# crowsonkb/style-transfer-pytorch

Measured on AMD Instinct MI355X. Metric: optimizer iterations/sec, higher is better.
Workload: dtype f32 (3x3 convs: fp16x3 split-plane MFMA, fp32 accumulate); 1 GPU; 512x512 single-scale hot loop (closure + Adam + clamp + EMA), 1 style image 512x512, VGG-19 synthetic weights, max pooling; parallelism=single GPU

## Files before the change

style-transfer-pytorch_amd/csrc/st_closure.hip:

```cpp
#include <cmath>
#include <cstdlib>
#include <mutex>

#include "st_plan.h"

namespace st {

void conv_arithmetic(const st_net* net, int conv, bool dgrad, ConvProblem& c) {
    const bool wide = dgrad ? net->wide_bwd[conv] : net->wide_fwd[conv];
    if (wide) {
        c.wgt_split = dgrad ? net->wsx_bwd[conv] : net->wsx_fwd[conv];
        c.planes = 3;
        c.elem = 0;
    } else {
        c.wgt_split = dgrad ? net->ws_bwd[conv] : net->ws_fwd[conv];
        c.planes = net->conv_planes;
        c.elem = net->conv_elem;
    }
}

int plan_alloc(st_plan* p, float** out, size_t floats) {
    void* ptr = nullptr;
    const size_t bytes = ((floats * sizeof(float) + 255) / 256) * 256;
    hipError_t e = hipMalloc(&ptr, bytes);
// ... 226 lines not shown
                StyleHead& h0 = p->head[0];
                static Option fwd_too("ST_CONV1_GRAM_IN_FORWARD", 0);
                p->gram1_fused = (fork_heads || fwd_too.get() != 0) && last_layer >= 1 && bounds && p->reference_taps && h0.allocated &&
                                 conv_first_gram_applies(p->H, p->W, image, n.y, h0.gram.max_splits);
                if (hbm_profiled(p, HBM_CONV1_FWD, (3 + 64) * hw4, s, [&] {
                        if (p->gram1_fused)
                            return launch_conv_first_fwd_gram(image, net->w_first, net->bias[0], n.y, p->H, p->W, s, n.y_amax,
                                                              h0.gram.partial, h0.gram.partial_sum, h0.gram.max_splits,
                                                              &p->gram1_splits, net->w_first_l1max, net->b_first_max);
                        return launch_conv_first_fwd(image, net->w_first, net->bias[0], n.y, p->H, p->W, s, nullptr, 0, 0,
                                                     bounds ? n.y_amax : nullptr);
                    }))
                    return 1;
            } else {
                ConvProblem c{};
                forward_conv(p, i, c);
                if (pool_follows(p, i, last_layer)) c.pool_out = p->pool[kProgram[i + 1].index].y;
                pooled_by_conv = fuse_pool(c, n, fork_heads, nullptr);
                if (conv_launch_profiled(p, c, s)) return 1;
            }
            prev = &n;
            if (fork_heads) {
                for (int k = 0; k < p->n_style; ++k)
                    if (p->style_op[k] == i) ST_HIP(hipEventRecord(p->tap_ready[k], s));
            }
        } else {
            Node& n = p->pool[op.index];
            if (!pooled_by_conv && launch_pool_fwd(prev->y, n.y, prev->c, prev->h, prev->w, net->pooling, s)) return 1;
            pooled_by_conv = false;
            prev = &n;
        }
    }
    return 0;
}

int ensure_moment_alloc(st_plan* p, StyleHead& h) {
    if (h.allocated) return 0;
    const size_t nn = (size_t)h.n * h.n;
    if (plan_alloc(p, &h.srm, nn) || plan_alloc(p, &h.ssym, nn) || plan_alloc(p, &h.mean, h.n) || plan_alloc(p, &h.bvec, h.n))
        return 1;
    long long splits = (16ll << 20) / (long long)nn;
    if (splits > 1024) splits = 1024;
    if (splits < 8) splits = 8;
    h.gram.max_splits = (int)splits;
    if (plan_alloc(p, &h.gram.partial, (size_t)splits * nn) ||
        plan_alloc(p, &h.gram.partial_sum, (size_t)splits * h.n))
        return 1;
    const long long wg = ((h.npix_local + 255) / 256) * (h.n / 64);
    if (wg < 512) {
        size_t need = (size_t)(h.n / 32) * h.n * (size_t)h.npix_local;
        if (need > kConvScratchFloats) need = kConvScratchFloats;
        if (plan_alloc(p, &h.conv_scratch, need)) return 1;
    }
    h.allocated = true;
    return 0;
}

int ensure_style_alloc(st_plan* p, StyleHead& h) {
    if (ensure_moment_alloc(p, h)) return 1;
    const size_t nn = (size_t)h.n * h.n;
    if (p->style_kind == 1) return h.gram_t ? 0 : plan_alloc(p, &h.gram_t, nn);
    if (h.w2_allocated) return 0;
    float** mats[] = {&h.cov_t, &h.root_t, &h.cov, &h.tmat, &h.mmat, &h.root, &h.gm, &h.dt, &h.dcov};
    for (float** m : mats)
        if (!*m && plan_alloc(p, m, nn)) return 1;
    if ((!h.mean_t && plan_alloc(p, &h.mean_t, h.n)) || (!h.gdiag && plan_alloc(p, &h.gdiag, 64))) return 1;
    float* nsbase = nullptr;
    if (plan_alloc(p, &nsbase, ns_workspace_floats(h.n))) return 1;
    ns_workspace_carve(h.ns, nsbase, h.n);
    if (ns_workspace_reset(h.ns, nullptr)) return 1;
// ... 20 lines not shown

HeadSite head_site(st_plan* p, int j) {
    HeadSite at;
    const int op = p->style_op[j];
    Node& tap = node_at(p, op);
    at.h = &p->head[op];
    at.tap = &tap;
    at.weight = p->style_weight[j];
    at.loss = p->losses + 1 + j;
    at.grad = tap.g;
    at.grad_amax = tap.g_amax;
    at.slot = j;
    return at;
}

int moments_of_tap(st_plan* p, const HeadSite& at, float* mean_out, float* srm_out, hipStream_t s, float* cov_out) {
    StyleHead& h = *at.h;
    const Node& tap = *at.tap;
    const int idx = at.slot;
    const bool fused = idx == 0 && p->gram1_fused;
    const int splits = fused ? p->gram1_splits : gram_choose_splits(h.n, h.npix_local, h.gram.max_splits);
    static Option gram_f32("ST_GRAM_F32", 0);
    auto gram = [&] {
        if (!fused && !(ablate_side() & 1) &&
            launch_gram_partial(tap.y, h.n, h.npix_local, splits, h.gram, s,
                                (p->net->conv_elem == 1 && !gram_f32.get()) ? tap.y_amax : nullptr))
            return 1;
        return launch_gram_finalize(h.gram, h.n, h.npix, splits, mean_out, srm_out, s, cov_out, kCovEps);
    };
    if (idx == 0 && !fused) return hbm_profiled(p, HBM_GRAM1, 4.0 * h.n * (double)h.npix_local, s, gram);
    return gram();
}

int moment_sums_of_tap(st_plan* p, int j, float* sums, hipStream_t s) {
    StyleHead& h = p->head[p->style_op[j]];
    const Node& tap = node_at(p, p->style_op[j]);
    const int splits = gram_choose_splits(h.n, h.npix_local, h.gram.max_splits);
    if (launch_gram_partial(tap.y, h.n, h.npix_local, splits, h.gram, s, p->net->conv_elem == 1 ? tap.y_amax : nullptr))
        return 1;
    return launch_gram_finalize(h.gram, h.n, 1, splits, sums + (size_t)h.n * h.n, sums, s);
}

GemmBatch one_gemm(int n, const float* a, const float* b, float* d, int ta, int tb) {
    GemmBatch g{};
    g.n = n; g.count = 1;
    g.p[0].a1 = a; g.p[0].b1 = b; g.p[0].d = d; g.p[0].ta1 = ta; g.p[0].tb1 = tb;
    g.p[0].epilogue = EPI_SCALE; g.p[0].c = 1.f;
    return g;
}

// ... 32 lines not shown
    if (launch_gemm_batch(mm, s)) return 1;
    const W2LossJob job{h.mean, h.mean_t, h.cov, h.cov_t, h.root, n, w, at.loss, h.gdiag};
    if (idx >= 0 && ns_chain_combined() && (ns_chain_mask() & (idx == 4 ? 4 : idx == 3 ? 2 : 1))) {
        const float* mm1[1] = {h.mmat};
        float* r1[1] = {h.root};
        float* g1[1] = {h.gm};
        NSWorkspace* w1[1] = {&h.ns};
        if (ns_chain_delayed() && idx != 4) ST_HIP(hipStreamWaitEvent(s, p->aux_fwd, 0));
        if (ns_sqrt_chain(mm1, r1, g1, &n, w1, &m_partials, &job, 1, s)) return 1;
        if (tl) ST_HIP(hipEventRecord(tlh[1], s));
    } else {
        int root_partials = 0;
        if (ns_sqrt_forward(h.mmat, h.root, n, h.ns, s, m_partials, &root_partials)) return 1;
        if (tl) ST_HIP(hipEventRecord(tlh[1], s));
        if (ns_sqrt_backward(h.root, nullptr, h.gdiag, h.gm, n, h.ns, s, &job, root_partials)) return 1;
    }
    if (tl) ST_HIP(hipEventRecord(tlh[2], s));
    if (launch_gemm_batch(one_gemm(n, h.gm, h.root_t, h.dt, 0, 1), s)) return 1;
    if (launch_gemm_batch(one_gemm(n, h.root_t, h.dt, h.dcov, 1, 0), s)) return 1;
    const bool f16 = p->net->conv_elem == 1;
    return launch_style_grad_finish(h.dcov, h.mean, h.mean_t, n, w, h.npix, h.ssym, h.bvec, s, f16 ? h.s_amax : nullptr);
}

int style_heads_shallow_lockstep(st_plan* p, hipStream_t s, const int* idx, int lanes) {
    const bool with_cov = gram_fused_cov();
    StyleHead* h[3];
    HeadSite at[3];
    int n[3];
    static Option defer_opt("ST_GRAM_DEFER_PIXELS", 0);
    const bool defer = defer_opt.get() > 0 && (long long)p->H * p->W >= defer_opt.get();
    for (int l = 0; l < lanes; ++l) {
        at[l] = head_site(p, idx[l]);
        h[l] = at[l].h;
        n[l] = h[l]->n;
        ST_HIP(hipStreamWaitEvent(s, defer ? p->aux_fwd : p->tap_ready[idx[l]], 0));
        if (moments_of_tap(p, at[l], h[l]->mean, h[l]->srm, s, with_cov ? h[l]->cov : nullptr)) return 1;
        if (!with_cov && launch_cov_from_moments(h[l]->mean, h[l]->srm, h[l]->cov, n[l], kCovEps, s)) return 1;
    }
    auto batch3 = [&](auto make) {
        GemmBatch g{};
        g.n = 64; g.count = lanes;
        for (int l = 0; l < lanes; ++l) g.n = std::max(g.n, n[l]);
        for (int l = 0; l < lanes; ++l) {
            g.p[l] = make(l);
            g.p[l].n = n[l];
        }
        return launch_gemm_batch(g, s);
    };
    if (batch3([&](int l) { return one_gemm(n[l], h[l]->root_t, h[l]->cov, h[l]->tmat, 0, 0).p[0]; })) return 1;
    if (batch3([&](int l) { return one_gemm(n[l], h[l]->tmat, h[l]->root_t, h[l]->mmat, 0, 0).p[0]; })) return 1;
    const float* mm[3] = {};
    float* roots[3] = {};
    NSWorkspace* ws[3] = {};
    for (int l = 0; l < lanes; ++l) { mm[l] = h[l]->mmat; roots[l] = h[l]->root; ws[l] = &h[l]->ns; }
    W2LossJob jobs[3];
    for (int l = 0; l < lanes; ++l)
        jobs[l] = W2LossJob{h[l]->mean, h[l]->mean_t, h[l]->cov, h[l]->cov_t, h[l]->root, n[l], at[l].weight, at[l].loss, h[l]->gdiag};
    const float* croots[3] = {};
// ... 41 lines not shown
        c.planes = 2; c.elem = 1; c.amax_word = tap.y_amax; c.wgt_amax = h.s_amax;
    }
    c.scratch = h.conv_scratch;
    if (idx == 4 && head5_masks_its_gradient()) c.out_mask = tap.y;
    if (ablate_side() & 2) return 0;
    const long long npix = (long long)tap.h * tap.w;
    if (head_dgrad_small_applies(n, npix))
        return hbm_profiled(p, HBM_HEAD_1X1, 2.0 * n * (double)npix * sizeof(float), s, [&] {
            return launch_head_dgrad_small(h.ssym, tap.y, h.bvec, c.out_mask, at.grad, n, npix, c.out_amax, s);
        });
    return hbm_profiled(p, HBM_HEAD_1X1, 2.0 * n * (double)tap.h * tap.w * sizeof(float), s, [&] { return launch_conv(c, s); });
}

bool op_is_tap(const st_plan* p, int op) {
    for (int i = 0; i < p->n_content; ++i)
        if (p->content_op[i] == op) return true;
    for (int k = 0; k < p->n_style; ++k)
        if (p->style_op[k] == op) return true;
    return false;
}

int join_head_for_conv(st_plan* p, int conv_index, hipStream_t s) {
    for (int k = 0; k < p->n_style; ++k) {
        if (!head_taps_conv(p, k, conv_index)) continue;
        ST_HIP(hipStreamWaitEvent(s, p->head_done[k], 0));
    }
    return 0;
}

void dgrad_conv(const st_plan* p, int i, ConvProblem& c) {
    const st_net* net = p->net;
    const OpDesc& op = kProgram[i];
    const OpDesc& pop = kProgram[i - 1];
    const Node& n = p->conv[op.index];
    const Node& in = node_at(p, i - 1);
    const bool top = i == kNumOps - 1;
    c.in = n.g; c.mask = (top && !head5_masks_its_gradient()) ? n.y : nullptr;
    c.out_mask = (pop.kind == 0) ? in.y : nullptr;
    c.wgt = net->w_bwd[op.index]; c.bias = nullptr; c.out = in.g;
    c.cin = op.cout; c.cout = op.cin; c.height = n.h; c.width = n.w; c.taps = 9; c.relu = 0;
    c.accumulate = (pop.kind == 0 && op_is_tap(p, i - 1)) ? 1 : 0;
    c.scratch = p->conv_scratch;
    conv_arithmetic(net, op.index, true, c);
    c.amax_word = n.g_amax; c.out_amax = net->conv_elem == 1 ? in.g_amax : nullptr;
}

int run_backward(st_plan* p, float* grad_image, hipStream_t s) {
// ... 99 lines not shown
    return 0;
}

int loss_and_grad(st_plan* p, const float* image, float* grad_out, float* losses_out, hipStream_t s) {
    if (require_targets(p) || ensure_grad_alloc(p)) return 1;
    if (ensure_streams(p, s)) return 1;
    if (p->timeline) ST_HIP(hipEventRecord(p->tl_start, s));
    auto tv = [&](hipStream_t ts) {
        return hbm_profiled(p, HBM_TV, 2.0 * 3 * 4.0 * p->H * p->W, ts, [&] {
            return launch_tv(image, p->H, p->W, p->tv_weight, grad_out, p->red_partials, p->losses + 6, ts, p->tickets + 0);
        });
    };
    static Option tv_slot_opt("ST_TV_SLOT", 0);
    const bool tv_tail = tv_slot_opt.get() == 1 && !p->aux_stream;
    if (!tv_tail) {
        const int tvk = shallow_heads_lockstep(p) ? 2 : 0;
        if (!p->aux_stream && ensure_head_stream(p, tvk)) return 1;
        hipStream_t tvs = p->aux_stream ? p->aux_stream : p->head_stream[tvk];
        ST_HIP(hipEventRecord(p->aux_in, s));
        ST_HIP(hipStreamWaitEvent(tvs, p->aux_in, 0));
        if (tv(tvs)) return 1;
        ST_HIP(hipEventRecord(p->tv_done, tvs));
    }
    if (run_forward(p, image, 29, s, true)) return 1;
    if (p->timeline) ST_HIP(hipEventRecord(p->tl_fwd, s));
    const int cop = p->content_op[0];
    Node& ct = node_at(p, cop);
    ST_HIP(hipEventRecord(p->aux_fwd, s));
    auto content = [&](hipStream_t cstream) {
        ST_HIP(hipStreamWaitEvent(cstream, p->aux_fwd, 0));
        if (hbm_profiled(p, HBM_CONTENT, 3.0 * 4.0 * ct.count(), cstream, [&] {
                return launch_content_mse(ct.y, p->content_target[cop], (long long)ct.count(), p->content_weight[0], ct.g,
                                          p->red_partials + 4 * kStreamBlocks, p->losses + 0, cstream, p->tickets + 64);
            }))
            return 1;
        ST_HIP(hipEventRecord(p->content_done, cstream));
        return 0;
    };
    if (p->aux_stream && content(p->aux_stream)) return 1;
    const bool lockstep = shallow_heads_lockstep(p);
    for (int k = 4; k >= (lockstep ? 3 : 0); --k) {
        const bool on_caller = k == 4 && p->head4_on_caller;
        if (!on_caller && ensure_head_stream(p, k)) return 1;
        hipStream_t hs = on_caller ? s : p->head_stream[k];
        if (!on_caller) ST_HIP(hipStreamWaitEvent(hs, p->tap_ready[k], 0));
        if (style_head(p, head_site(p, k), hs)) return 1;
        ST_HIP(hipEventRecord(p->head_done[k], hs));
        if (p->timeline) ST_HIP(hipEventRecord(p->tl_head[k], hs));
        if (k == 3 && !p->aux_stream && content(p->head_stream[3])) return 1;
    }
    if (lockstep) {
        const int three[3] = {2, 1, 0};
        if (ensure_head_stream(p, 2) || style_heads_shallow_lockstep(p, p->head_stream[2], three, 3)) return 1;
    }
    if (tv_tail) {
        hipStream_t tvs = p->head_stream[lockstep ? 2 : 0];
        if (tv(tvs)) return 1;
        ST_HIP(hipEventRecord(p->tv_done, tvs));
    }
    if (run_backward(p, grad_out, s)) return 1;
    if (!p->defer_sum && launch_sum_losses(p->losses, s, losses_out)) return 1;
    if (p->timeline) {
        ST_HIP(hipEventRecord(p->tl_bwd, s));
        if (++p->tl_count % 10 == 0) {
            ST_HIP(hipEventSynchronize(p->tl_bwd));
            float f = 0, b = 0, h[5] = {};
            hipEventElapsedTime(&f, p->tl_start, p->tl_fwd);
            hipEventElapsedTime(&b, p->tl_start, p->tl_bwd);
            for (int i = 0; i < 5; ++i) hipEventElapsedTime(&h[i], p->tl_start, p->tl_head[i]);
            float c4[3] = {};
            for (int i = 0; i < 3; ++i) hipEventElapsedTime(&c4[i], p->tl_start, p->tl_h4[i]);
            fprintf(stderr, "[timeline] relu5_1 head: moments known %.3f | NS forward done %.3f | NS backward done %.3f | gradient written %.3f ms\n",
                    c4[0], c4[1], c4[2], h[4]);
            float c3[3] = {};
            for (int i = 0; i < 3; ++i) hipEventElapsedTime(&c3[i], p->tl_start, p->tl_h3[i]);
// ... 56 lines not shown
```

style-transfer-pytorch_amd/csrc/st_common.h:

```cpp
#pragma once

#include <hip/hip_runtime.h>

#include <algorithm>
#include <atomic>
#include <cstdarg>
#include <cstdio>
#include <string>

namespace st {

typedef float f32x16 __attribute__((ext_vector_type(16)));
typedef float f32x4 __attribute__((ext_vector_type(4)));
typedef float f32x2 __attribute__((ext_vector_type(2)));

constexpr int kWave = 64;

void set_error(const char* fmt, ...);
const char* get_error();

#define ST_HIP(expr)                                                                           \
    do {                                                                                       \
        hipError_t _e = (expr);                                                                \
        if (_e != hipSuccess) {                                                                \
// ... 40 lines not shown
        const unsigned long long c = cached.load(std::memory_order_acquire);
        if ((unsigned)(c >> 32) == g) return (int)(unsigned)(c & 0xffffffffull);
        const int v = option_lookup(name, dflt);
        cached.store(((unsigned long long)g << 32) | (unsigned)v, std::memory_order_release);
        return v;
    }
};

__device__ __forceinline__ float wave_sum(float v) {
#pragma unroll
    for (int off = 32; off > 0; off >>= 1) v += __shfl_xor(v, off, 64);
    return v;
}

__device__ __forceinline__ float block_sum_256(float v, float* scratch) {
    v = wave_sum(v);
    const int lane = threadIdx.x & 63, wave = threadIdx.x >> 6;
    if (lane == 0) scratch[wave] = v;
    __syncthreads();
    float r = 0.f;
    if (threadIdx.x == 0) r = (scratch[0] + scratch[1]) + (scratch[2] + scratch[3]);
    __syncthreads();
    return r;
}

struct W2LossJob {
    const float *mean, *mean_t, *cov, *cov_t, *root;
    int n;
    float weight;
    float* loss_out;
    float* gdiag_out;
};
__device__ __forceinline__ float w2_gdiag(const W2LossJob& j) { return -2.f * (j.weight / (float)j.n); }
__device__ __forceinline__ void w2_loss_block(const W2LossJob& j, float* scratch) {
#pragma clang fp contract(off)
    float sm = 0.f, sc = 0.f;
    for (int i = threadIdx.x; i < j.n; i += 256) {
        const float d = j.mean[i] - j.mean_t[i];
        sm += d * d;
        const size_t ii = (size_t)i * j.n + i;
        sc += (j.cov_t[ii] + j.cov[ii]) - 2.f * j.root[ii];
    }
    sm = block_sum_256(sm, scratch);
    sc = block_sum_256(sc, scratch);
    if (threadIdx.x == 0) {
        const float fn = (float)j.n;
// ... 139 lines not shown

int launch_pool_fwd(const float* in, float* out, int channels, int height, int width, int mode, hipStream_t s);
bool conv_pc_fuses_pool(const ConvProblem& p);
int fold_halo_amax(const ConvProblem& p, hipStream_t stream);
struct PcOverlap {
    int rows_b;
    int rows_bottom;
    int shape_i, tw_i;
    int shape_b, tw_b;
    double cost_split, cost_whole;
    bool pays;
    bool pool;
};
bool conv_pc_overlap_choice(const ConvProblem& p, PcOverlap* out);
int launch_pool_bwd_codes(const unsigned char* code, const float* grad_out, float* grad_in, int channels, int height,
                          int width, hipStream_t s);
int launch_pool_bwd(const float* in, const float* grad_out, float* grad_in, int channels, int height,
                    int width, int mode, hipStream_t s);

struct GramWorkspace {
    float* partial;
    float* partial_sum;
    int max_splits;
};
int gram_choose_splits(int channels, long long npix, int max_splits);
int launch_gram_partial(const float* feat, int channels, long long npix, int splits, GramWorkspace ws,
                        hipStream_t s, const unsigned int* bound = nullptr);
int launch_gram_finalize(GramWorkspace ws, int channels, long long npix, int splits, float* mean, float* srm,
                         hipStream_t s, float* cov = nullptr, float cov_eps = 0.f);

enum GemmEpilogue {
    EPI_SCALE = 0,
    EPI_IDENT_MINUS = 1,
    EPI_DIFF = 2,
    EPI_DEV_SQRT_SCALE = 3
};
struct GemmProblem {
    const float* a1; const float* b1;
    const float* a2; const float* b2; const float* b2sub;
    float* d;
    int ta1, tb1, ta2;
    int epilogue;
    float c, ci;
    const float* dev_scalar;
    int n;
    float* sumsq_partials;
};
bool gemm_sumsq_fusable(int n);
struct GemmBatch {
    GemmProblem p[6];
    int count;
    int n;
// ... 220 lines not shown
```

style-transfer-pytorch_amd/csrc/st_gram.hip:

```cpp
#include "st_common.h"

namespace st {
namespace {

constexpr int GT = 64;
constexpr int GK = 64;
constexpr int GP = 68;
constexpr int HK = 32;
constexpr int HP = 40;

typedef _Float16 f16x8 __attribute__((ext_vector_type(8)));

__device__ __forceinline__ void tile_pair(int block, int tiles, int& ti, int& tj) {
    int t = block, row = 0, len = tiles;
    while (t >= len) {
        t -= len;
        --len;
        ++row;
    }
    ti = row;
    tj = row + t;
}

__device__ __forceinline__ void store_tile_pair(float* __restrict__ out, int C, int ti, int tj, int wi, int wj,
// ... 94 lines not shown
            const f32x4 a = *reinterpret_cast<const f32x4*>(la + kb * 8);
            const f32x4 b = *reinterpret_cast<const f32x4*>(lb + kb * 8);
#pragma unroll
            for (int e = 0; e < 4; ++e) acc = __builtin_amdgcn_mfma_f32_32x32x2f32(a[e], b[e], acc, 0, 0, 0);
        }
        if (more) store_tile(buf ^ 1);
        __syncthreads();
    }

    store_tile_pair(partial + (size_t)split * C * C, C, ti, tj, wi, wj, l31, half, acc);
    if (diag) {
#pragma unroll
        for (int r = 0; r < 4; ++r) {
            float v = rowsum[r];
            v += __shfl_xor(v, 1, 64);
            v += __shfl_xor(v, 2, 64);
            v += __shfl_xor(v, 4, 64);
            v += __shfl_xor(v, 8, 64);
            if ((tid & 15) == 0) partial_sum[(size_t)split * C + ti * GT + srow + 16 * r] = v;
        }
    }
}

__global__ __launch_bounds__(256) void gram_partial_f16_kernel(const float* __restrict__ feat, int C, long long N,
                                                               int splits, long long per_split,
                                                               const unsigned int* __restrict__ bound,
                                                               float* __restrict__ partial,
                                                               float* __restrict__ partial_sum, int xcd_remap) {
    __shared__ __attribute__((aligned(16))) _Float16 lds[2][2][2][GT * HP];
    const int tid = threadIdx.x, lane = tid & 63;
    const int wave = __builtin_amdgcn_readfirstlane(tid >> 6);
    const int l31 = lane & 31, half = lane >> 5;
    const int wi = wave >> 1, wj = wave & 1;
    const int tiles = C / GT;
    int ti, tj;
    const unsigned int lb = logical_block(xcd_remap);
    tile_pair((int)(lb % gridDim.x), tiles, ti, tj);
    const int split = (int)(lb / gridDim.x);
    const long long k_begin = split * per_split;
    const long long k_end = (k_begin + per_split < N) ? k_begin + per_split : N;
    const bool diag = (ti == tj);
    const bool vec_ok = (N % 4 == 0);
    const int ex = scale_exp(amax_read(bound));
    const float scale = pow2f(ex), unscale = pow2f(-ex);

    const int srow = tid >> 2, scol = (tid & 3) * 8;
    float va[8], vb[8];
    float rowsum = 0.f;

    auto load_row = [&](const float* p, long long k, float (&v)[8]) {
#pragma unroll
        for (int q = 0; q < 2; ++q) {
            if (vec_ok && k + 4 * q + 3 < k_end) {
                const f32x4 t = *reinterpret_cast<const f32x4*>(p + 4 * q);
#pragma unroll
                for (int e = 0; e < 4; ++e) v[4 * q + e] = t[e];
            } else {
#pragma unroll
                for (int e = 0; e < 4; ++e) v[4 * q + e] = (k + 4 * q + e < k_end) ? p[4 * q + e] : 0.f;
            }
        }
    };
    auto load_tile = [&](long long k0) {
        const long long k = k0 + scol;
        load_row(feat + (size_t)(ti * GT + srow) * N + k, k, va);
        if (!diag) load_row(feat + (size_t)(tj * GT + srow) * N + k, k, vb);
    };
    auto split_store = [&](const float (&v)[8], _Float16* p0, _Float16* p1) {
        f16x8 h0, h1;
#pragma unroll
        for (int e = 0; e < 8; ++e) {
            const float x = v[e] * scale;
            const _Float16 a = (_Float16)x;
            h0[e] = a;
            h1[e] = (_Float16)(x - (float)a);
        }
        *reinterpret_cast<f16x8*>(p0) = h0;
        *reinterpret_cast<f16x8*>(p1) = h1;
    };
    auto store_tile = [&](int buf) {
        const int off = srow * HP + scol;
        split_store(va, &lds[buf][0][0][off], &lds[buf][0][1][off]);
        if (!diag) split_store(vb, &lds[buf][1][0][off], &lds[buf][1][1][off]);
        rowsum += ((va[0] + va[1]) + (va[2] + va[3])) + ((va[4] + va[5]) + (va[6] + va[7]));
    };

    f32x16 acc;
#pragma unroll
    for (int r = 0; r < 16; ++r) acc[r] = 0.f;

    const long long span = k_end - k_begin;
    const int nstages = span > 0 ? (int)((span + HK - 1) / HK) : 0;
    if (nstages > 0) {
        load_tile(k_begin);
        store_tile(0);
    }
    __syncthreads();
    const int ob = diag ? 0 : 1;
    for (int st = 0; st < nstages; ++st) {
        const int buf = st & 1;
        const bool more = st + 1 < nstages;
        if (more) load_tile(k_begin + (long long)(st + 1) * HK);
        const int aoff = (wi * 32 + l31) * HP + 8 * half, boff = (wj * 32 + l31) * HP + 8 * half;
#pragma unroll
        for (int kb = 0; kb < HK / 16; ++kb) {
            const f16x8 a0 = *reinterpret_cast<const f16x8*>(&lds[buf][0][0][aoff + kb * 16]);
            const f16x8 a1 = *reinterpret_cast<const f16x8*>(&lds[buf][0][1][aoff + kb * 16]);
// ... 2 lines not shown
            acc = __builtin_amdgcn_mfma_f32_32x32x16_f16(a0, b0, acc, 0, 0, 0);
            acc = __builtin_amdgcn_mfma_f32_32x32x16_f16(a0, b1, acc, 0, 0, 0);
            acc = __builtin_amdgcn_mfma_f32_32x32x16_f16(a1, b0, acc, 0, 0, 0);
        }
        if (more) store_tile(buf ^ 1);
        __syncthreads();
    }
#pragma unroll
    for (int r = 0; r < 16; ++r) acc[r] = acc[r] * unscale * unscale;
    float* out = partial + (size_t)split * C * C;
    if (diag) {
        float* t = reinterpret_cast<float*>(&lds[0][0][0][0]);
#pragma unroll
        for (int r = 0; r < 16; ++r)
            t[(wi * 32 + (r & 3) + 8 * (r >> 2) + 4 * half) * 65 + wj * 32 + l31] = acc[r];
        __syncthreads();
        for (int idx = tid; idx < GT * GT; idx += 256) {
            const int row = idx >> 6, col = idx & 63;
            out[(size_t)(ti * GT + row) * C + ti * GT + col] = row <= col ? t[row * 65 + col] : t[col * 65 + row];
        }
    } else {
        store_tile_pair(out, C, ti, tj, wi, wj, l31, half, acc);
    }
    if (diag) {
        float v = rowsum;
        v += __shfl_xor(v, 1, 64);
        v += __shfl_xor(v, 2, 64);
        if ((tid & 3) == 0) partial_sum[(size_t)split * C + ti * GT + srow] = v;
    }
}

__global__ __launch_bounds__(256, 2) void gram_partial_f16_wide_kernel(const float* __restrict__ feat, int C, long long N,
                                                                       int splits, long long per_split,
                                                                       const unsigned int* __restrict__ bound,
                                                                       float* __restrict__ partial,
                                                                       float* __restrict__ partial_sum, int xcd_remap) {
    constexpr int TS = 128;
    __shared__ __attribute__((aligned(16))) _Float16 lds[2][2][TS * HP];
    const int tid = threadIdx.x, lane = tid & 63;
    const int wave = __builtin_amdgcn_readfirstlane(tid >> 6);
    const int l31 = lane & 31, half = lane >> 5;
    const int wi = wave >> 1, wj = wave & 1;
    int ti, tj;
    const unsigned int lb = logical_block(xcd_remap);
    tile_pair((int)(lb % gridDim.x), C / TS, ti, tj);
    const int split = (int)(lb / gridDim.x);
    const long long k_begin = split * per_split;
    const long long k_end = (k_begin + per_split < N) ? k_begin + per_split : N;
    const bool diag = (ti == tj);
    const bool vec_ok = (N % 4 == 0);
    const int ex = scale_exp(amax_read(bound));
// ... 196 lines not shown
    if (want > by_len) want = by_len;
    if (want > max_splits) want = max_splits;
    if (want < 1) want = 1;
    return (int)want;
}

int launch_gram_partial(const float* feat, int channels, long long npix, int splits, GramWorkspace ws,
                        hipStream_t s, const unsigned int* bound) {
    ST_REQUIRE(channels % GT == 0, "gram: channel count must be a multiple of 64");
    ST_REQUIRE(splits >= 1 && splits <= ws.max_splits, "gram: bad split count %d", splits);
    long long per_split = (npix + splits - 1) / splits;
    per_split = (per_split + 3) & ~3ll;
    static Option remap_opt("ST_XCD_REMAP", 1);
    const int remap = remap_opt.get();
    if (bound && gram_wide_tiles(channels, npix)) {
        const int wide = (channels / 128) * (channels / 128 + 1) / 2;
        hipLaunchKernelGGL(gram_partial_f16_wide_kernel, dim3(wide, splits), dim3(256), 0, s, feat, channels, npix, splits,
                           per_split, bound, ws.partial, ws.partial_sum, remap);
        ST_LAUNCH_CHECK();
        return 0;
    }
    const int tiles = (channels / GT) * (channels / GT + 1) / 2;
    if (bound)
        hipLaunchKernelGGL(gram_partial_f16_kernel, dim3(tiles, splits), dim3(256), 0, s, feat, channels, npix,
                           splits, per_split, bound, ws.partial, ws.partial_sum, remap);
    else
        hipLaunchKernelGGL(gram_partial_kernel, dim3(tiles, splits), dim3(256), 0, s, feat, channels, npix,
                           splits, per_split, ws.partial, ws.partial_sum, remap);
    ST_LAUNCH_CHECK();
    return 0;
}

int launch_gram_finalize(GramWorkspace ws, int channels, long long npix, int splits, float* mean, float* srm,
                         hipStream_t s, float* cov, float cov_eps) {
    const long long total = (long long)channels * channels + channels;
    const int blocks = (int)((total + 31) / 32);
    hipLaunchKernelGGL(gram_finalize_kernel, dim3(blocks), dim3(256), 0, s, ws.partial, ws.partial_sum,
                       channels, npix, splits, mean, srm, cov, cov_eps);
    ST_LAUNCH_CHECK();
    return 0;
}

}
```

style-transfer-pytorch_amd/csrc/st_plan.h:

```cpp
#pragma once

#include <functional>
#include <unordered_map>
#include <vector>

#include "../../include/st_amd.h"
#include "st_common.h"

namespace st {

struct OpDesc {
    int kind;
    int index;
    int feat_index;
    int cin, cout;
};
const OpDesc kProgram[] = {
    {0, 0, 1, 3, 64},     {0, 1, 3, 64, 64},    {1, 0, 4, 64, 64},    {0, 2, 6, 64, 128},
    {0, 3, 8, 128, 128},  {1, 1, 9, 128, 128},  {0, 4, 11, 128, 256}, {0, 5, 13, 256, 256},
    {0, 6, 15, 256, 256}, {0, 7, 17, 256, 256}, {1, 2, 18, 256, 256}, {0, 8, 20, 256, 512},
    {0, 9, 22, 512, 512}, {0, 10, 24, 512, 512}, {0, 11, 26, 512, 512}, {1, 3, 27, 512, 512},
    {0, 12, 29, 512, 512},
};
constexpr int kNumOps = sizeof(kProgram) / sizeof(kProgram[0]);
// ... 124 lines not shown
    hipStream_t chain_stream = nullptr;
    hipEvent_t moments_ready[5] = {}, chain_done[5] = {};
    hipEvent_t pack_done = nullptr, halo_landed = nullptr;
    unsigned int* halo_bound = nullptr;

    int rank = 0, world = 1;
    float* head_result[5] = {};
    struct Phase {
        std::function<int(hipStream_t)> run;
        st_exchange ex;
        const float* halo = nullptr;
    };
    std::unordered_map<const float*, bool> halo_inline;
    std::vector<Phase> phases;
    size_t phase_pos = 0;
    const float* ph_image = nullptr;
    float* ph_grad = nullptr;
    int ph_last_layer = -1;
    unsigned ph_option_gen = 0;
    hipStream_t head_stream[5] = {};
    bool head_stream_owned[5] = {};
    hipEvent_t tap_ready[5] = {};
    hipEvent_t head_done[5] = {};
    bool streams_ready = false;
    int device = 0;
    bool graph_enabled = false;
    hipStream_t main_stream = nullptr;
    bool gram1_fused = false;
    int gram1_splits = 0;
    bool compact_streams = false;
    bool head4_on_caller = false;
    std::vector<hipStream_t> junk_streams;
    hipEvent_t bridge_in = nullptr, bridge_out = nullptr;
    hipStream_t aux_stream = nullptr;
    hipEvent_t aux_in = nullptr, aux_fwd = nullptr, tv_done = nullptr, content_done = nullptr;
    hipGraph_t graph = nullptr;
    hipGraphExec_t graph_exec = nullptr;
    const float* gk_image = nullptr;
    float* gk_grad = nullptr;
    float* gk_losses = nullptr;
    int gk_seen = 0;
    bool capturing = false;
    bool timeline = false;
    hipEvent_t tl_start = nullptr, tl_fwd = nullptr, tl_head[5] = {}, tl_bwd = nullptr;
    hipEvent_t tl_h4[4] = {};
    hipEvent_t tl_h3[4] = {};
// ... 85 lines not shown
```

style-transfer-pytorch_amd/csrc/st_pointwise.hip:

```cpp
#include "st_common.h"

namespace st {
namespace {

__global__ void fill_kernel(float* p, long long n, float v) {
    for (long long i = blockIdx.x * 256ll + threadIdx.x; i < n; i += (long long)gridDim.x * 256) p[i] = v;
}
__global__ void identity_kernel(float* p, int n) {
    const long long nn = (long long)n * n;
    for (long long i = blockIdx.x * 256ll + threadIdx.x; i < nn; i += (long long)gridDim.x * 256)
        p[i] = ((int)(i / n) == (int)(i % n)) ? 1.f : 0.f;
}

__global__ void cov_kernel(const float* __restrict__ mean, const float* __restrict__ srm,
                           float* __restrict__ cov, int n, float eps) {
#pragma clang fp contract(off)
    const long long nn = (long long)n * n;
    for (long long i = blockIdx.x * 256ll + threadIdx.x; i < nn; i += (long long)gridDim.x * 256) {
        const int r = (int)(i / n), c = (int)(i % n);
        const float outer = mean[r] * mean[c];
        const float d = srm[i] - outer;
        cov[i] = d + ((r == c) ? eps : 0.f);
    }
}
// ... 49 lines not shown
                                                         float* __restrict__ norm_out, float* __restrict__ a_scaled,
                                                         const float* __restrict__ g, const float* __restrict__ gdiag,
                                                         float* __restrict__ second, int n, int mode, W2LossJob loss) {
    __shared__ float scratch[4];
    __shared__ float norm_sh;
    float s = 0.f;
    for (int i = threadIdx.x; i < nparts; i += 256) s += partials[i];
    s = block_sum_256(s, scratch);
    if (threadIdx.x == 0) {
        norm_sh = sqrtf(s);
        if (blockIdx.x == 0) norm_out[0] = norm_sh;
    }
    __syncthreads();
    const float d = norm_sh;
    const float dv = (mode == 2) ? (loss.loss_out ? w2_gdiag(loss) : gdiag[0]) / d : 1.f;
    const long long nn = (long long)n * n;
    for (long long i = blockIdx.x * 256ll + threadIdx.x; i < nn; i += (long long)gridDim.x * 256) {
        const float y = a[i] / d;
        a_scaled[i] = y;
        const bool diag = (int)(i / n) == (int)(i % n);
        second[i] = (mode == 3) ? ((diag ? 3.f : 0.f) - y) * 0.5f : (mode == 1) ? g[i] / d : (diag ? dv : 0.f);
    }
    if (loss.loss_out && blockIdx.x == 0) w2_loss_block(loss, scratch);
}

struct LastBlock {
    unsigned int* ticket;
};
__device__ __forceinline__ bool last_block_arrives(const LastBlock& lb, bool* shared_flag) {
    if (lb.ticket == nullptr) return false;
    if (threadIdx.x == 0) {
        __builtin_amdgcn_fence(__ATOMIC_RELEASE, "agent");
        asm volatile("s_waitcnt vmcnt(0)" ::: "memory");
        const unsigned int prev = atomicAdd(lb.ticket, 1u);
        const bool last = (prev == gridDim.x - 1);
        if (last) *lb.ticket = 0u;
        *shared_flag = last;
    }
    __syncthreads();
    const bool last = *shared_flag;
    if (last) __builtin_amdgcn_fence(__ATOMIC_ACQUIRE, "agent");
    return last;
}

template <bool ACC>
__global__ __launch_bounds__(256) void content_mse_kernel(const float* __restrict__ feat,
                                                          const float* __restrict__ target, long long count,
                                                          float weight, float norm, float* __restrict__ grad,
                                                          float* __restrict__ partials, LastBlock lb,
                                                          float final_count, float* __restrict__ loss_out) {
#pragma clang fp contract(off)
    __shared__ float scratch[4];
    __shared__ bool is_last;
    float s = 0.f;
    if ((count & 3) == 0) {
        const long long n4 = count >> 2;
        const f32x4* f4 = reinterpret_cast<const f32x4*>(feat);
        const f32x4* t4 = reinterpret_cast<const f32x4*>(target);
        f32x4* g4 = reinterpret_cast<f32x4*>(grad);
        for (long long i = blockIdx.x * 256ll + threadIdx.x; i < n4; i += (long long)gridDim.x * 256) {
            const f32x4 f = f4[i], t = t4[i];
            f32x4 g;
            if (ACC) g = g4[i];
#pragma unroll
            for (int k = 0; k < 4; ++k) {
// ... 772 lines not shown
```

Before: 457.4 it/s.

## Fuse gram finalize into partial kernel via last-block tickets; skip redundant stream events

Adds a one-launch gram path in which each split block of a tile pair writes its partial and row sums, and the last arriving block (tracked by a per-pair atomic ticket) reduces the splits and writes mean, second-moment and covariance, including the mirrored tile. This removes the separate finalize launch. The fused path is gated by the ST_GRAM_ONE_LAUNCH option, which defaults to 0. Separately, in plain single-stream mode it skips recording and waiting on tap_ready and head_done events for heads that run inline on the caller stream or whose taps are already ordered, which trims event overhead.

New measurement: 458.2 it/s (median of 5 runs). Within noise of the previous version (+0.2%).

```diff
diff --git a/style-transfer-pytorch_amd/csrc/st_closure.hip b/style-transfer-pytorch_amd/csrc/st_closure.hip
--- a/style-transfer-pytorch_amd/csrc/st_closure.hip
+++ b/style-transfer-pytorch_amd/csrc/st_closure.hip
@@ -272,7 +272,7 @@
             prev = &n;
             if (fork_heads) {
                 for (int k = 0; k < p->n_style; ++k)
-                    if (p->style_op[k] == i) ST_HIP(hipEventRecord(p->tap_ready[k], s));
+                    if (p->style_op[k] == i && !p->tap_unwaited[k]) ST_HIP(hipEventRecord(p->tap_ready[k], s));
             }
         } else {
             Node& n = p->pool[op.index];
@@ -296,6 +296,14 @@
     if (plan_alloc(p, &h.gram.partial, (size_t)splits * nn) ||
         plan_alloc(p, &h.gram.partial_sum, (size_t)splits * h.n))
         return 1;
+    if (h.n % 64 == 0 && h.n / 64 >= kGramOneLaunchTiles) {
+        const size_t pairs = (size_t)(h.n / 64) * (h.n / 64 + 1) / 2;
+        float* words = nullptr;
+        if (plan_alloc(p, &words, pairs) || plan_alloc(p, &h.gram.pair_sums, pairs * kGramOneLaunchSplits * 128)) return 1;
+        ST_HIP(hipMemset(words, 0, pairs * sizeof(unsigned int)));
+        ST_HIP(hipStreamSynchronize(nullptr));
+        h.gram.tickets = reinterpret_cast<unsigned int*>(words);
+    }
     const long long wg = ((h.npix_local + 255) / 256) * (h.n / 64);
     if (wg < 512) {
         size_t need = (size_t)(h.n / 32) * h.n * (size_t)h.npix_local;
@@ -362,10 +370,9 @@
     const int splits = fused ? p->gram1_splits : gram_choose_splits(h.n, h.npix_local, h.gram.max_splits);
     static Option gram_f32("ST_GRAM_F32", 0);
     auto gram = [&] {
-        if (!fused && !(ablate_side() & 1) &&
-            launch_gram_partial(tap.y, h.n, h.npix_local, splits, h.gram, s,
-                                (p->net->conv_elem == 1 && !gram_f32.get()) ? tap.y_amax : nullptr))
-            return 1;
+        if (!fused && !(ablate_side() & 1))
+            return launch_gram_moments(tap.y, h.n, h.npix_local, h.npix, splits, h.gram, mean_out, srm_out, s,
+                                       (p->net->conv_elem == 1 && !gram_f32.get()) ? tap.y_amax : nullptr, cov_out, kCovEps);
         return launch_gram_finalize(h.gram, h.n, h.npix, splits, mean_out, srm_out, s, cov_out, kCovEps);
     };
     if (idx == 0 && !fused) return hbm_profiled(p, HBM_GRAM1, 4.0 * h.n * (double)h.npix_local, s, gram);
@@ -444,18 +451,22 @@
     return launch_style_grad_finish(h.dcov, h.mean, h.mean_t, n, w, h.npix, h.ssym, h.bvec, s, f16 ? h.s_amax : nullptr);
 }
 
+static bool gram_deferred(const st_plan* p) {
+    static Option defer_opt("ST_GRAM_DEFER_PIXELS", 0);
+    return defer_opt.get() > 0 && (long long)p->H * p->W >= defer_opt.get();
+}
+
 int style_heads_shallow_lockstep(st_plan* p, hipStream_t s, const int* idx, int lanes) {
     const bool with_cov = gram_fused_cov();
     StyleHead* h[3];
     HeadSite at[3];
     int n[3];
-    static Option defer_opt("ST_GRAM_DEFER_PIXELS", 0);
-    const bool defer = defer_opt.get() > 0 && (long long)p->H * p->W >= defer_opt.get();
+    const bool defer = gram_deferred(p);
     for (int l = 0; l < lanes; ++l) {
         at[l] = head_site(p, idx[l]);
         h[l] = at[l].h;
         n[l] = h[l]->n;
-        ST_HIP(hipStreamWaitEvent(s, defer ? p->aux_fwd : p->tap_ready[idx[l]], 0));
+        if (defer || !p->tap_unwaited[idx[l]]) ST_HIP(hipStreamWaitEvent(s, defer ? p->aux_fwd : p->tap_ready[idx[l]], 0));
         if (moments_of_tap(p, at[l], h[l]->mean, h[l]->srm, s, with_cov ? h[l]->cov : nullptr)) return 1;
         if (!with_cov && launch_cov_from_moments(h[l]->mean, h[l]->srm, h[l]->cov, n[l], kCovEps, s)) return 1;
     }
@@ -543,7 +554,7 @@
 
 int join_head_for_conv(st_plan* p, int conv_index, hipStream_t s) {
     for (int k = 0; k < p->n_style; ++k) {
-        if (!head_taps_conv(p, k, conv_index)) continue;
+        if (!head_taps_conv(p, k, conv_index) || p->head_inline[k]) continue;
         ST_HIP(hipStreamWaitEvent(s, p->head_done[k], 0));
     }
     return 0;
@@ -689,6 +700,15 @@
         if (tv(tvs)) return 1;
         ST_HIP(hipEventRecord(p->tv_done, tvs));
     }
+    const bool lockstep = shallow_heads_lockstep(p);
+    const int three[3] = {2, 1, 0};
+    const bool plain = !p->aux_stream && !p->capturing && !p->timeline;
+    for (int k = 0; k < 5; ++k) {
+        p->head_inline[k] = plain && k == 4 && p->head4_on_caller;
+        p->tap_unwaited[k] = p->head_inline[k];
+    }
+    if (plain && lockstep && !gram_deferred(p))
+        for (int l = 1; l < 3; ++l) p->tap_unwaited[three[l]] = p->style_op[three[l]] < p->style_op[three[0]];
     if (run_forward(p, image, 29, s, true)) return 1;
     if (p->timeline) ST_HIP(hipEventRecord(p->tl_fwd, s));
     const int cop = p->content_op[0];
@@ -705,19 +725,17 @@
         return 0;
     };
     if (p->aux_stream && content(p->aux_stream)) return 1;
-    const bool lockstep = shallow_heads_lockstep(p);
     for (int k = 4; k >= (lockstep ? 3 : 0); --k) {
         const bool on_caller = k == 4 && p->head4_on_caller;
         if (!on_caller && ensure_head_stream(p, k)) return 1;
         hipStream_t hs = on_caller ? s : p->head_stream[k];
         if (!on_caller) ST_HIP(hipStreamWaitEvent(hs, p->tap_ready[k], 0));
         if (style_head(p, head_site(p, k), hs)) return 1;
-        ST_HIP(hipEventRecord(p->head_done[k], hs));
+        if (!p->head_inline[k]) ST_HIP(hipEventRecord(p->head_done[k], hs));
         if (p->timeline) ST_HIP(hipEventRecord(p->tl_head[k], hs));
         if (k == 3 && !p->aux_stream && content(p->head_stream[3])) return 1;
     }
     if (lockstep) {
-        const int three[3] = {2, 1, 0};
         if (ensure_head_stream(p, 2) || style_heads_shallow_lockstep(p, p->head_stream[2], three, 3)) return 1;
     }
     if (tv_tail) {
diff --git a/style-transfer-pytorch_amd/csrc/st_common.h b/style-transfer-pytorch_amd/csrc/st_common.h
--- a/style-transfer-pytorch_amd/csrc/st_common.h
+++ b/style-transfer-pytorch_amd/csrc/st_common.h
@@ -86,6 +86,28 @@
     if (threadIdx.x == 0) r = (scratch[0] + scratch[1]) + (scratch[2] + scratch[3]);
     __syncthreads();
     return r;
+}
+
+struct LastBlock {
+    unsigned int* ticket;
+};
+__device__ __forceinline__ bool last_block_arrives(const LastBlock& lb, unsigned int arrivals, bool* shared_flag) {
+    if (lb.ticket == nullptr) return false;
+    if (threadIdx.x == 0) {
+        __builtin_amdgcn_fence(__ATOMIC_RELEASE, "agent");
+        asm volatile("s_waitcnt vmcnt(0)" ::: "memory");
+        const unsigned int prev = atomicAdd(lb.ticket, 1u);
+        const bool last = (prev == arrivals - 1);
+        if (last) *lb.ticket = 0u;
+        *shared_flag = last;
+    }
+    __syncthreads();
+    const bool last = *shared_flag;
+    if (last) __builtin_amdgcn_fence(__ATOMIC_ACQUIRE, "agent");
+    return last;
+}
+__device__ __forceinline__ bool last_block_arrives(const LastBlock& lb, bool* shared_flag) {
+    return last_block_arrives(lb, gridDim.x, shared_flag);
 }
 
 struct W2LossJob {
@@ -271,12 +293,19 @@
     float* partial;
     float* partial_sum;
     int max_splits;
-};
+    unsigned int* tickets;
+    float* pair_sums;
+};
+constexpr int kGramOneLaunchTiles = 8;
+constexpr int kGramOneLaunchSplits = 32;
 int gram_choose_splits(int channels, long long npix, int max_splits);
 int launch_gram_partial(const float* feat, int channels, long long npix, int splits, GramWorkspace ws,
                         hipStream_t s, const unsigned int* bound = nullptr);
 int launch_gram_finalize(GramWorkspace ws, int channels, long long npix, int splits, float* mean, float* srm,
                          hipStream_t s, float* cov = nullptr, float cov_eps = 0.f);
+bool gram_one_launch_applies(int channels, long long npix, int splits, GramWorkspace ws, const unsigned int* bound);
+int launch_gram_moments(const float* feat, int channels, long long npix_local, long long npix, int splits, GramWorkspace ws,
+                        float* mean, float* srm, hipStream_t s, const unsigned int* bound, float* cov, float cov_eps);
 
 enum GemmEpilogue {
     EPI_SCALE = 0,
diff --git a/style-transfer-pytorch_amd/csrc/st_gram.hip b/style-transfer-pytorch_amd/csrc/st_gram.hip
--- a/style-transfer-pytorch_amd/csrc/st_gram.hip
+++ b/style-transfer-pytorch_amd/csrc/st_gram.hip
@@ -140,12 +140,126 @@
     }
 }
 
+struct GramFinish {
+    unsigned int* tickets;
+    float* pair_sums;
+    float* mean;
+    float* srm;
+    float* cov;
+    float n, eps;
+};
+constexpr int FT = GT * 65;
+constexpr int kFinishLdsFloats = 2 * FT + 2 * GT + 1;
+
+__device__ __forceinline__ float tree8(const float (&r)[8]) {
+#pragma clang fp contract(off)
+    return ((r[0] + r[1]) + (r[2] + r[3])) + ((r[4] + r[5]) + (r[6] + r[7]));
+}
+
+__device__ __forceinline__ void gram_finish_pair(const GramFinish& f, const float* partial, int C, int splits, int pair,
+                                                 int ti, int tj, float* lds) {
+#pragma clang fp contract(off)
+    const int tid = threadIdx.x;
+    float* t_srm = lds;
+    float* t_cov = lds + FT;
+    float* means = lds + 2 * FT;
+    const size_t total = (size_t)C * C;
+    const bool diag = ti == tj;
+    if (tid < 2 * GT) {
+        const float* src = f.pair_sums + (size_t)pair * kGramOneLaunchSplits * 2 * GT + tid;
+        float v[kGramOneLaunchSplits];
+#pragma unroll
+        for (int k = 0; k < kGramOneLaunchSplits; ++k) v[k] = src[(size_t)(k < splits ? k : splits - 1) * 2 * GT];
+        float r[8];
+#pragma unroll
+        for (int g = 0; g < 8; ++g) r[g] = 0.f;
+#pragma unroll
+        for (int k = 0; k < kGramOneLaunchSplits; ++k) r[k & 7] += (k < splits) ? v[k] : 0.f;
+        const float m = tree8(r) / f.n;
+        means[tid] = m;
+        if (diag && tid < GT) f.mean[ti * GT + tid] = m;
+    }
+    __syncthreads();
+#pragma unroll
+    for (int q0 = 0; q0 < 4; q0 += 2) {
+        f32x4 r[2][8];
+#pragma unroll
+        for (int qq = 0; qq < 2; ++qq)
+#pragma unroll
+            for (int g = 0; g < 8; ++g) r[qq][g] = f32x4{0.f, 0.f, 0.f, 0.f};
+        for (int k0 = 0; k0 < splits; k0 += 8) {
+            f32x4 v[2][8];
+#pragma unroll
+            for (int qq = 0; qq < 2; ++qq) {
+                const int qi = (q0 + qq) * 256 + tid;
+                const float* src = partial + (size_t)(ti * GT + (qi >> 4)) * C + tj * GT + 4 * (qi & 15);
+#pragma unroll
+                for (int j = 0; j < 8; ++j)
+                    v[qq][j] = *reinterpret_cast<const f32x4*>(src + (size_t)(k0 + j < splits ? k0 + j : splits - 1) * total);
+            }
+#pragma unroll
+            for (int qq = 0; qq < 2; ++qq)
+#pragma unroll
+                for (int j = 0; j < 8; ++j) {
+                    const bool live = k0 + j < splits;
+#pragma unroll
+                    for (int e = 0; e < 4; ++e) r[qq][j][e] += live ? v[qq][j][e] : 0.f;
+                }
+        }
+#pragma unroll
+        for (int qq = 0; qq < 2; ++qq) {
+            const int qi = (q0 + qq) * 256 + tid;
+            const int row = qi >> 4, col = 4 * (qi & 15);
+            const int grow = ti * GT + row, gcol = tj * GT + col;
+            const float mean_r = means[row];
+            f32x4 t, c;
+#pragma unroll
+            for (int e = 0; e < 4; ++e) {
+                const float sh[8] = {r[qq][0][e], r[qq][1][e], r[qq][2][e], r[qq][3][e],
+                                     r[qq][4][e], r[qq][5][e], r[qq][6][e], r[qq][7][e]};
+                t[e] = tree8(sh) / f.n;
+                const float outer = mean_r * means[(diag ? 0 : GT) + col + e];
+                const float d = t[e] - outer;
+                c[e] = d + ((grow == gcol + e) ? f.eps : 0.f);
+            }
+            *reinterpret_cast<f32x4*>(f.srm + (size_t)grow * C + gcol) = t;
+            if (f.cov) *reinterpret_cast<f32x4*>(f.cov + (size_t)grow * C + gcol) = c;
+            if (!diag) {
+#pragma unroll
+                for (int e = 0; e < 4; ++e) {
+                    t_srm[row * 65 + col + e] = t[e];
+                    t_cov[row * 65 + col + e] = c[e];
+                }
+            }
+        }
+    }
+    if (diag) return;
+    __syncthreads();
+#pragma unroll
+    for (int q = 0; q < 4; ++q) {
+        const int qi = q * 256 + tid;
+        const int mrow = qi >> 4, mcol = 4 * (qi & 15);
+        f32x4 t, c;
+#pragma unroll
+        for (int e = 0; e < 4; ++e) {
+            t[e] = t_srm[(mcol + e) * 65 + mrow];
+            c[e] = t_cov[(mcol + e) * 65 + mrow];
+        }
+        const size_t at = (size_t)(tj * GT + mrow) * C + ti * GT + mcol;
+        *reinterpret_cast<f32x4*>(f.srm + at) = t;
+        if (f.cov) *reinterpret_cast<f32x4*>(f.cov + at) = c;
+    }
+}
+
+template <bool FIN>
 __global__ __launch_bounds__(256) void gram_partial_f16_kernel(const float* __restrict__ feat, int C, long long N,
                                                                int splits, long long per_split,
                                                                const unsigned int* __restrict__ bound,
                                                                float* __restrict__ partial,
-                                                               float* __restrict__ partial_sum, int xcd_remap) {
+                                                               float* __restrict__ partial_sum, int xcd_remap,
+                                                               GramFinish fin) {
     __shared__ __attribute__((aligned(16))) _Float16 lds[2][2][2][GT * HP];
+    static_assert(sizeof(lds) >= kFinishLdsFloats * sizeof(float), "the finisher borrows the staging buffers");
     const int tid = threadIdx.x, lane = tid & 63;
     const int wave = __builtin_amdgcn_readfirstlane(tid >> 6);
     const int l31 = lane & 31, half = lane >> 5;
@@ -153,7 +267,8 @@
     const int tiles = C / GT;
     int ti, tj;
     const unsigned int lb = logical_block(xcd_remap);
-    tile_pair((int)(lb % gridDim.x), tiles, ti, tj);
+    const int pair = (int)(lb % gridDim.x);
+    tile_pair(pair, tiles, ti, tj);
     const int split = (int)(lb / gridDim.x);
     const long long k_begin = split * per_split;
     const long long k_end = (k_begin + per_split < N) ? k_begin + per_split : N;
@@ -164,7 +279,7 @@
 
     const int srow = tid >> 2, scol = (tid & 3) * 8;
     float va[8], vb[8];
-    float rowsum = 0.f;
+    float rowsum = 0.f, rowsum_b = 0.f;
 
     auto load_row = [&](const float* p, long long k, float (&v)[8]) {
 #pragma unroll
@@ -201,6 +316,7 @@
         split_store(va, &lds[buf][0][0][off], &lds[buf][0][1][off]);
         if (!diag) split_store(vb, &lds[buf][1][0][off], &lds[buf][1][1][off]);
         rowsum += ((va[0] + va[1]) + (va[2] + va[3])) + ((va[4] + va[5]) + (va[6] + va[7]));
+        if (FIN && !diag) rowsum_b += ((vb[0] + vb[1]) + (vb[2] + vb[3])) + ((vb[4] + vb[5]) + (vb[6] + vb[7]));
     };
 
     f32x16 acc;
@@ -249,11 +365,30 @@
     } else {
         store_tile_pair(out, C, ti, tj, wi, wj, l31, half, acc);
     }
-    if (diag) {
+    if (diag || FIN) {
         float v = rowsum;
         v += __shfl_xor(v, 1, 64);
         v += __shfl_xor(v, 2, 64);
-        if ((tid & 3) == 0) partial_sum[(size_t)split * C + ti * GT + srow] = v;
+        if (diag && (tid & 3) == 0) partial_sum[(size_t)split * C + ti * GT + srow] = v;
+        if (FIN) {
+            float w = rowsum_b;
+            w += __shfl_xor(w, 1, 64);
+            w += __shfl_xor(w, 2, 64);
+            float* ps = fin.pair_sums + ((size_t)pair * kGramOneLaunchSplits + split) * 2 * GT;
+            if ((tid & 3) == 0) {
+                ps[srow] = v;
+                ps[GT + srow] = diag ? v : w;
+            }
+        }
+    }
+    if (FIN) {
+        asm volatile("s_waitcnt vmcnt(0)" ::: "memory");
+        __syncthreads();
+        float* fl = reinterpret_cast<float*>(&lds[0][0][0][0]);
+        if (!last_block_arrives(LastBlock{fin.tickets + pair}, (unsigned int)splits,
+                                reinterpret_cast<bool*>(fl + kFinishLdsFloats - 1)))
+            return;
+        gram_finish_pair(fin, partial, C, splits, pair, ti, tj, fl);
     }
 }
 
@@ -496,8 +631,8 @@
     }
     const int tiles = (channels / GT) * (channels / GT + 1) / 2;
     if (bound)
-        hipLaunchKernelGGL(gram_partial_f16_kernel, dim3(tiles, splits), dim3(256), 0, s, feat, channels, npix,
-                           splits, per_split, bound, ws.partial, ws.partial_sum, remap);
+        hipLaunchKernelGGL(gram_partial_f16_kernel<false>, dim3(tiles, splits), dim3(256), 0, s, feat, channels, npix,
+                           splits, per_split, bound, ws.partial, ws.partial_sum, remap, GramFinish{});
     else
         hipLaunchKernelGGL(gram_partial_kernel, dim3(tiles, splits), dim3(256), 0, s, feat, channels, npix,
                            splits, per_split, ws.partial, ws.partial_sum, remap);
@@ -515,4 +650,28 @@
     return 0;
 }
 
-}
+bool gram_one_launch_applies(int channels, long long npix, int splits, GramWorkspace ws, const unsigned int* bound) {
+    static Option opt("ST_GRAM_ONE_LAUNCH", 0);
+    return opt.get() != 0 && bound != nullptr && ws.tickets != nullptr && ws.pair_sums != nullptr && channels % GT == 0 &&
+           channels / GT >= kGramOneLaunchTiles && splits <= kGramOneLaunchSplits && !gram_wide_tiles(channels, npix);
+}
+
+int launch_gram_moments(const float* feat, int channels, long long npix_local, long long npix, int splits, GramWorkspace ws,
+                        float* mean, float* srm, hipStream_t s, const unsigned int* bound, float* cov, float cov_eps) {
+    if (!gram_one_launch_applies(channels, npix_local, splits, ws, bound)) {
+        if (launch_gram_partial(feat, channels, npix_local, splits, ws, s, bound)) return 1;
+        return launch_gram_finalize(ws, channels, npix, splits, mean, srm, s, cov, cov_eps);
+    }
+    ST_REQUIRE(splits >= 1 && splits <= ws.max_splits, "gram: bad split count %d", splits);
+    long long per_split = (npix_local + splits - 1) / splits;
+    per_split = (per_split + 3) & ~3ll;
+    static Option remap_opt("ST_XCD_REMAP", 1);
+    const int tiles = (channels / GT) * (channels / GT + 1) / 2;
+    const GramFinish fin{ws.tickets, ws.pair_sums, mean, srm, cov, (float)npix, cov_eps};
+    hipLaunchKernelGGL(gram_partial_f16_kernel<true>, dim3(tiles, splits), dim3(256), 0, s, feat, channels, npix_local,
+                       splits, per_split, bound, ws.partial, ws.partial_sum, remap_opt.get(), fin);
+    ST_LAUNCH_CHECK();
+    return 0;
+}
+
+}
diff --git a/style-transfer-pytorch_amd/csrc/st_plan.h b/style-transfer-pytorch_amd/csrc/st_plan.h
--- a/style-transfer-pytorch_amd/csrc/st_plan.h
+++ b/style-transfer-pytorch_amd/csrc/st_plan.h
@@ -170,6 +170,8 @@
     bool head_stream_owned[5] = {};
     hipEvent_t tap_ready[5] = {};
     hipEvent_t head_done[5] = {};
+    bool tap_unwaited[5] = {};
+    bool head_inline[5] = {};
     bool streams_ready = false;
     int device = 0;
     bool graph_enabled = false;
diff --git a/style-transfer-pytorch_amd/csrc/st_pointwise.hip b/style-transfer-pytorch_amd/csrc/st_pointwise.hip
--- a/style-transfer-pytorch_amd/csrc/st_pointwise.hip
+++ b/style-transfer-pytorch_amd/csrc/st_pointwise.hip
@@ -95,25 +95,6 @@
         second[i] = (mode == 3) ? ((diag ? 3.f : 0.f) - y) * 0.5f : (mode == 1) ? g[i] / d : (diag ? dv : 0.f);
     }
     if (loss.loss_out && blockIdx.x == 0) w2_loss_block(loss, scratch);
-}
-
-struct LastBlock {
-    unsigned int* ticket;
-};
-__device__ __forceinline__ bool last_block_arrives(const LastBlock& lb, bool* shared_flag) {
-    if (lb.ticket == nullptr) return false;
-    if (threadIdx.x == 0) {
-        __builtin_amdgcn_fence(__ATOMIC_RELEASE, "agent");
-        asm volatile("s_waitcnt vmcnt(0)" ::: "memory");
-        const unsigned int prev = atomicAdd(lb.ticket, 1u);
-        const bool last = (prev == gridDim.x - 1);
-        if (last) *lb.ticket = 0u;
-        *shared_flag = last;
-    }
-    __syncthreads();
-    const bool last = *shared_flag;
-    if (last) __builtin_amdgcn_fence(__ATOMIC_ACQUIRE, "agent");
-    return last;
 }
 
 template <bool ACC>
```
